# LiChaiUSTC/Speech-enhancement-based-on-a-maximum-likelihood-criterion

Hardware: AMD Instinct MI355X
Metric: training frames/sec (128-frame minibatch) (higher is better)
Workload: dtype f32

## Files before the change

### speech-enhancement-based-on-a-maximum-likelihood-criterion_amd/__init__.py

```python
import collections
import ctypes as C
import os
import subprocess

import numpy as np

_HERE = os.path.dirname(os.path.abspath(__file__))
_CSRC = os.path.join(_HERE, "csrc")
LIB_PATH = os.path.join(_CSRC, "libmlggd.so")
MAXLAYER = 10
UNIQUE_ID_BYTES = 128

_fp = C.POINTER(C.c_float)
_fpp = C.POINTER(_fp)


class MlggdError(RuntimeError):
    pass


class _ConfigSlots(C.Union):
    _fields_ = [("mask_bins", C.c_int32), ("reserved", C.c_int32 * 5)]


# ... 32 lines not shown
    "mlggd_debug_stamp_select", "mlggd_debug_stamp_read",
    "mlggd_load_frames", "mlggd_train_frames", "mlggd_train_frames_async", "mlggd_cv_all_frames", "mlggd_forward_frames",
    "mlggd_alloc_pinned", "mlggd_alloc_pinned_on", "mlggd_free_pinned", "mlggd_set_cv_device_reduce",
    "mlggd_comm_info", "mlggd_debug_plan_count", "mlggd_debug_buffers", "mlggd_debug_math", "mlggd_debug_out_slabs", "mlggd_debug_gemm_plan",
    "mlggd_debug_keep_ranks", "mlggd_debug_rank_tensor",
    "mlggd_wave_to_lps", "mlggd_lps_to_wave", "mlggd_enhance_wave",
    "mlggd_enhance_waves_layout", "mlggd_enhance_waves",
    "mlggd_score_waves", "mlggd_enhance_waves_scored",
    "mlggd_stoi_layout", "mlggd_stoi_waves", "mlggd_enhance_waves_scored_stoi",
    "mlggd_live_layout", "mlggd_live_open", "mlggd_live_push", "mlggd_live_received", "mlggd_live_close",
    "mlggd_error_stats", "mlggd_error_stats_frames", "mlggd_ggd_fit",
    "mlggd_set_shapefactors", "mlggd_get_shapefactors", "mlggd_read_shapefactors",
    "mlggd_output_stats", "mlggd_output_stats_frames", "mlggd_gv_fit", "mlggd_set_gv", "mlggd_get_gv", "mlggd_read_gv",
    "mlggd_wave_samples", "mlggd_mix_waves", "mlggd_lps_stats", "mlggd_norm_from_stats",
    "mlggd_load_waves", "mlggd_cv_all_waves", "mlggd_set_noise", "mlggd_train_waves",
    "mlggd_load_frames_nat", "mlggd_train_frames_nat", "mlggd_cv_all_frames_nat", "mlggd_forward_frames_nat",
    "mlggd_nat_estimate", "mlggd_nat_rows", "mlggd_get_nat_frames",
    "mlggd_set_mask", "mlggd_get_mask", "mlggd_get_mask_bins", "mlggd_mask_targets", "mlggd_mask_select",
    "mlggd_set_asymmetry", "mlggd_get_asymmetry", "mlggd_error_stats_signed", "mlggd_error_stats_signed_frames",
    "mlggd_asym_fit", "mlggd_read_asymmetry",
    "mlggd_set_scale_mode", "mlggd_get_scale_mode", "mlggd_get_scale_state", "mlggd_set_scale_state",
    "mlggd_read_scale_state", "mlggd_write_scale_state",
    "mlggd_rbm_open", "mlggd_rbm_set_rates", "mlggd_rbm_train_chunk", "mlggd_rbm_train_frames", "mlggd_rbm_visible_bias",
    "mlggd_rbm_debug_tensor", "mlggd_rbm_close", "mlggd_rbm_draws",
]
MAX_BETAS = 32

_lib = None


def build(force=False):
    srcs = [os.path.join(_CSRC, f) for f in ("engine.hip", "kernels.hip.h", "kernels64.hip.h", "spectral.hip.h", "score.hip.h", "live.hip.h",
                                             "live_rule.h", "stoi.hip.h", "stoi_rule.h", "colstats.hip.h", "gv_rule.h", "mask_rule.h", "mask.hip.h", "mix.hip.h",
                                             "mix_rule.h", "nat_rule.h", "rbm_rule.h", "rbm.hip.h", "asym_rule.h", "scale_rule.h", "devbuf.h", "devbuf_rule.h")]
    srcs.append(os.path.join(_HERE, "..", "include", "mlggd.h"))
    srcs.append(os.path.join(_HERE, "host", "errmodel.h"))
    srcs.append(os.path.join(_HERE, "host", "gvfile.h"))
    srcs.append(os.path.join(_HERE, "host", "asymfile.h"))
    srcs.append(os.path.join(_HERE, "host", "scalefile.h"))
    srcs.append(os.path.join(_HERE, "host", "binfile.h"))
    stale = not os.path.exists(LIB_PATH) or any(
        os.path.getmtime(LIB_PATH) < os.path.getmtime(s) for s in srcs)
    if force or stale:
        subprocess.check_call(["make", "-C", _CSRC, "-s"])
    return LIB_PATH


def load():
    global _lib
    if _lib is not None:
        return _lib
    if not os.path.exists(LIB_PATH):
        raise MlggdError("HIP extension %s is missing: run __graft_entry__.build() "
                         "(there is no CPU fallback)" % LIB_PATH)
    L = C.CDLL(LIB_PATH)
    L.mlggd_last_error.restype = C.c_char_p
    L.mlggd_gamma.restype = C.c_float
    L.mlggd_gamma.argtypes = [C.c_float]
    L.mlggd_create.argtypes = [C.POINTER(_Config), _fpp, _fpp, C.POINTER(C.c_void_p)]
    L.mlggd_destroy.argtypes = [C.c_void_p]
    L.mlggd_device_count.argtypes = [C.POINTER(C.c_int)]
    L.mlggd_train_chunk.argtypes = [C.c_void_p, C.c_int, _fp, _fp, C.POINTER(C.c_int)]
    L.mlggd_load_chunk.argtypes = [C.c_void_p, C.c_int, _fp, _fp]
    L.mlggd_train_resident.argtypes = [C.c_void_p, C.c_int, C.c_int, C.POINTER(C.c_int)]
    L.mlggd_sync.argtypes = [C.c_void_p]
    for f in (L.mlggd_cv_sqerr, L.mlggd_cv_abserr, L.mlggd_cv_loglik):
        f.argtypes = [C.c_void_p, C.c_int, _fp, _fp, _fp]
# ... 1291 lines not shown
```

### speech-enhancement-based-on-a-maximum-likelihood-criterion_amd/csrc/engine.hip

```cpp
#include <hip/hip_runtime.h>
#include <hip/hip_ext.h>

#include <dlfcn.h>
#include <math.h>
#include <stdarg.h>
#include <stdio.h>
#include <stdlib.h>
#include <string.h>

#include <algorithm>
#include <functional>
#include <mutex>
#include <string>
#include <vector>

#include "../../include/mlggd.h"
#include "../host/errmodel.h"
#include "../host/gvfile.h"
#include "../host/asymfile.h"
#include "../host/scalefile.h"
#include "kernels.hip.h"
#include "spectral.hip.h"
#include "score.hip.h"
#include "stoi.hip.h"
// ... 247 lines not shown
    int ar_shard = 1;
    hipEvent_t ev_grad[MLGGD_MAXLAYER] = {0}, ev_red[MLGGD_MAXLAYER] = {0}, ev_bias = nullptr, ev_bias_red = nullptr;

    hipEvent_t ev_t0 = nullptr, ev_t1 = nullptr;
    int last_steps = 0;
    bool timing_valid = false;
    int prof_class = -1, prof_layer = 0, prof_stride = 1;
    std::vector<hipEvent_t> prof_ev;
    size_t prof_used = 0, prof_cap = 0;
    hipEvent_t *prof_attach = nullptr;
    bool prof_attached = false;
    hipEvent_t stop_ev_next = nullptr;
    bool stop_ev_attached = false;
    int dp_stopev = 1;
    double prof_flops = 0, prof_bytes = 0;

    int stamp_class = -1, stamp_layer = 0, stamp_blocks = 0;
    DevBuf<long long> stamp_buf;

    struct DwpTable {
        DwpJobs key;
        bool fused;
        int grid;
        DevBuf<DwpDesc> dev;
    };
    std::vector<DwpTable> dwp_tables;
    std::vector<void *> allocs;
    std::vector<const void *> lds_attr_done;

    int mask_bins = 0;
    int mask_mode = mask_rule::kSelect;
    float mask_lo = mask_rule::kLo, mask_hi = mask_rule::kHi, mask_scale = mask_rule::kScale;
    int rbm_open = 0;
};

static long long *stamps_for(mlggd_engine *e, int cls, int layer, int blocks) {
    if (e->stamp_class != cls || e->stamp_layer != layer || !e->stamp_buf.p) return nullptr;
    if ((size_t)blocks * 8 > e->stamp_buf.cap) return nullptr;
    e->stamp_class = -1;
    e->stamp_blocks = blocks;
    return e->stamp_buf.p;
}

struct DevBufs {
    std::vector<void *> p;
    ~DevBufs() {
        for (void *q : p) hipFree(q);
    }
    template <typename T>
    int alloc(T **out, size_t count) {
        void *q = nullptr;
        HIPCHK(hipMalloc(&q, (count ? count : 1) * sizeof(T)));
        p.push_back(q);
        *out = (T *)q;
        return MLGGD_OK;
    }
    template <typename T>
    int upload(T **out, const T *host, size_t count) {
        CHK(alloc(out, count));
        if (count) HIPCHK(hipMemcpy(*out, host, count * sizeof(T), hipMemcpyHostToDevice));
        return MLGGD_OK;
    }
};

static int dev_alloc(mlggd_engine *e, float **p, size_t count) {
    const size_t bytes = (count + 64) * sizeof(float);
// ... 411 lines not shown
        if (a.Np >= (1 << 17)) return fail(MLGGD_ERR_ARG, "dW tile table: layer of %d units is too wide", a.Np);
        for (int tl = 0; tl < a.ntiles; tl++, n++) {
            const int kt = a.k_first + tl / a.n_wg, nt = tl % a.n_wg;
            const int k0 = kt * 64, n0 = nt * 64;
            DwpDesc &d = recs[n];
            d.A = a.Yrow + (k0 - a.k_base);
            d.Bm = a.dEdX + n0;
            const size_t base = (size_t)k0 * a.Np + n0;
            int rows = a.K - k0;
            rows = rows < 0 ? 0 : rows > 64 ? 64 : rows;
            if (a.wd_off) {
                rows = 0;
                d.W = a.Wt;
                d.D = a.delta;
                d.szW = 0;
            } else {
                d.W = (fused ? a.Wt : a.G) + base;
                d.D = fused ? a.delta + base : nullptr;
                const size_t to_end = ((size_t)a.Kp * a.Np - base) * sizeof(float);
                const size_t to_row = (size_t)rows * a.Np * sizeof(float);
                d.szW = (unsigned)(to_end < to_row ? to_end : to_row);
            }
            const int colsw = a.Np - n0 < 64 ? a.Np - n0 : 64;
            int nbias = (a.do_bias && kt == 0) ? a.N - n0 : 0;
            nbias = nbias < 0 ? 0 : nbias > 64 ? 64 : nbias;
            d.bias = (fused ? a.bias : a.gb) + n0;
            d.dbias = fused ? a.dbias + n0 : nullptr;
            d.ldA = a.ldA;
            d.Np = a.Np;
            d.packed = (unsigned)rows | ((unsigned)colsw << 8) | ((unsigned)nbias << 16) | (1u << 24);
        }
    }
    if (n != (size_t)J.total) return fail(MLGGD_ERR_STATE, "dW tile table: %zu records for %d tiles", n, J.total);
    for (; n < recs.size(); n++) {
        DwpDesc &d = recs[n];
        d = recs[0];
        d.packed = 0;
        d.szW = 0;
    }
    mlggd_engine::DwpTable t;
    t.key = key;
    t.fused = fused;
    t.grid = grid;
    HIPCHK(t.dev.grow(recs.size(), recs.size(), e->bufs, nullptr, nullptr));
    HIPCHK(hipMemcpy(t.dev.p, recs.data(), recs.size() * sizeof(DwpDesc), hipMemcpyHostToDevice));
    *out = t.dev.p;
    e->dwp_tables.push_back(std::move(t));
    return MLGGD_OK;
}

template <int H>
static int launch_dwp_t(mlggd_engine *e, const DwpJobs &J, bool fused, hipStream_t st, int stamp_layer) {
    const size_t lds = dwp_lds_floats() * sizeof(float);
    const int grid = dwp_grid(e, J.total);
    if (J.total < 1) return MLGGD_OK;
    const DwpDesc *table = nullptr;
    DwpConst C;
    C.B = J.job[0].B;
    C.nf = J.job[0].nf;
    C.mom = J.job[0].mom;
    C.lr = J.job[0].lr;
    C.wc = J.job[0].wc;
    bool bias_only = J.njobs > 0, any_bias_only = false;
    for (int j = 0; j < J.njobs; j++) {
        bias_only = bias_only && J.job[j].wd_off != 0;
        any_bias_only = any_bias_only || J.job[j].wd_off != 0;
    }
    if (any_bias_only) {
        if (!bias_only || !fused) return fail(MLGGD_ERR_STATE, "bias-only jobs need a launch of their own on the fused path");
        CHK(dwp_table(e, J, fused, grid, &table));
        unsigned nb;
        memcpy(&nb, &C.nf, sizeof(nb));
        if ((nb & 0x007FFFFFu) == 0u && C.nf >= 1.0f) {
            CHK(ensure_lds(e, k_dwp_bias<H, true>, lds));
            hipLaunchKernelGGL((k_dwp_bias<H, true>), dim3(grid), dim3(256), lds, st, table, J.total, C, (long long *)nullptr);
        } else {
            CHK(ensure_lds(e, k_dwp_bias<H, false>, lds));
            hipLaunchKernelGGL((k_dwp_bias<H, false>), dim3(grid), dim3(256), lds, st, table, J.total, C, (long long *)nullptr);
        }
        return launch_check("k_dwp_bias");
    }
    CHK(dwp_table(e, J, fused, grid, &table));
    if constexpr (H == 2 || H == 8) {
        if (e->stamp_class == KC_DW && e->stamp_layer == -1 && e->stamp_buf.p && fused && C.nf == 128.0f) {
            long long *sp = stamps_for(e, KC_DW, -1, 2 * grid);
            if (sp) {
                CHK(ensure_lds(e, k_dwp_phases<H>, lds));
                hipLaunchKernelGGL((k_dwp_phases<H>), dim3(grid), dim3(256), lds, st, table, J.total, C, sp);
                return launch_check("k_dwp_phases");
            }
        }
    }
    if constexpr (H == 2) {
        static const int abl = getenv("MLGGD_DWP_ABLATE") ? atoi(getenv("MLGGD_DWP_ABLATE")) : 0;
        if (abl && fused) {
#define DWP_ABL(A_)                                                                                       \
    case A_:                                                                                              \
        CHK(ensure_lds(e, k_dwp_ablate<H, A_>, lds));                                                     \
        launch_timed(e, k_dwp_ablate<H, A_>, dim3(grid), dim3(256), lds, st, table, J.total, C, (long long *)nullptr); \
        return launch_check("k_dwp_ablate");
            switch (abl) {
                DWP_ABL(1) DWP_ABL(2) DWP_ABL(3) DWP_ABL(4) DWP_ABL(7) DWP_ABL(15) DWP_ABL(31) DWP_ABL(63) DWP_ABL(16) DWP_ABL(48) DWP_ABL(256) DWP_ABL(1024) DWP_ABL(2048) DWP_ABL(512) DWP_ABL(576)
            default: return fail(MLGGD_ERR_ARG, "MLGGD_DWP_ABLATE=%d is not built", abl);
            }
#undef DWP_ABL
        }
    }
    long long *stamps = stamps_for(e, KC_DW, stamp_layer, grid);
    unsigned nfbits;
    memcpy(&nfbits, &C.nf, sizeof(nfbits));
    const bool pow2 = (nfbits & 0x007FFFFFu) == 0u && C.nf >= 1.0f;
#define DWP_LAUNCH(FUSED_, POW2_)                                                                         \
    {                                                                                                     \
        if (stamps) {                                                                                     \
            CHK(ensure_lds(e, k_dwp<H, FUSED_, POW2_, true>, lds));                                       \
            launch_timed(e, k_dwp<H, FUSED_, POW2_, true>, dim3(grid), dim3(256), lds, st, table, J.total, C, stamps); \
        } else {                                                                                          \
            CHK(ensure_lds(e, k_dwp<H, FUSED_, POW2_>, lds));                                             \
            launch_timed(e, k_dwp<H, FUSED_, POW2_>, dim3(grid), dim3(256), lds, st, table, J.total, C, stamps); \
        }                                                                                                 \
    }
    if (fused && pow2) DWP_LAUNCH(true, true)
    else if (fused) DWP_LAUNCH(true, false)
    else if (pow2) DWP_LAUNCH(false, true)
    else DWP_LAUNCH(false, false)
#undef DWP_LAUNCH
    return launch_check("k_dwp");
}
static bool dwp_usable(const mlggd_engine *e) {
    const int Hh = e->Bp / 64;
    return e->dw_persist && e->Bp % 64 == 0 && (Hh == 1 || Hh == 2 || Hh == 4 || Hh == 8);
}
static int launch_dwp(mlggd_engine *e, const DwpJobs &J, bool fused, hipStream_t st, int stamp_layer, int units = 0) {
    switch (units > 0 ? units : e->Bp / 64) {
    case 1: return launch_dwp_t<1>(e, J, fused, st, stamp_layer);
    case 2: return launch_dwp_t<2>(e, J, fused, st, stamp_layer);
    case 4: return launch_dwp_t<4>(e, J, fused, st, stamp_layer);
    case 8: return launch_dwp_t<8>(e, J, fused, st, stamp_layer);
    case 16: return launch_dwp_t<16>(e, J, fused, st, stamp_layer);
    default: return fail(MLGGD_ERR_STATE, "no dW kernel for %d units per tile", units);
    }
}

static bool gather_usable(const mlggd_engine *e, int world) {
    const long frames = (long)world * e->Bp;
    const long units = frames / 64;
    return e->dw_persist && e->B == e->Bp && frames % 64 == 0 &&
           (units == 1 || units == 2 || units == 4 || units == 8 || units == 16);
}
static int gather_alloc(mlggd_engine *e) {
    const size_t rows = (size_t)e->world * e->Bp;
    for (int l = 0; l < e->L - 1; l++) {
        const size_t width = e->dp_a2a ? (size_t)e->shard_rows[l + 1] * 64 : (size_t)e->lsp[l];
        CHK(dev_alloc(e, &e->Yall[l], rows * width));
        if (e->dp_a2a) {
            if (l == 0) {
                CHK(dev_alloc(e, &e->in_bunch_buf[0], rows * width));
                CHK(dev_alloc(e, &e->in_bunch_buf[1], rows * width));
                e->in_bunch = e->in_bunch_buf[0];
// ... 732 lines not shown
    if (ceil32(cfg->bunchsize) > 1152)
        return fail(MLGGD_ERR_ARG, "bunchsize %d too large for the loss kernel's LDS tile (max 1152)", cfg->bunchsize);
    int ndev = 0;
    hipError_t de = hipGetDeviceCount(&ndev);
    if (de != hipSuccess || ndev < 1)
        return fail(MLGGD_ERR_DEVICE, "no HIP device available (%s)", de == hipSuccess ? "count 0" : hipGetErrorString(de));
    if (cfg->device < 0 || cfg->device >= ndev)
        return fail(MLGGD_ERR_ARG, "GPU Num %d Not In Range %d-%d", cfg->device, 0, ndev - 1);

    mlggd_engine *e = new mlggd_engine();
    e->cfg = *cfg;
    e->L = cfg->numlayers;
    e->device = cfg->device;
    for (int i = 0; i < e->L; i++) {
        e->ls[i] = cfg->layersizes[i];
        e->lsp[i] = ceil32(cfg->layersizes[i]);
    }
    e->B = cfg->bunchsize;
    e->Bp = ceil32(e->B);
    e->K0 = e->ls[0];
    e->D = e->ls[e->L - 1];
    e->Dp = e->lsp[e->L - 1];
    e->nat_frames = cfg->nat_frames;
    e->mask_bins = cfg->mask_bins;
    if (const char *v = getenv("MLGGD_FWD_NW")) e->fwd_nw = atoi(v);
    if (const char *v = getenv("MLGGD_WAVES_LOOKUP")) e->ww.lookup_table = !strcmp(v, "table");
    if (const char *v = getenv("MLGGD_DX_NW")) e->dx_nw = atoi(v);
    if (const char *v = getenv("MLGGD_FWD_PIPE")) e->fwd_pipe = atoi(v);
    if (const char *v = getenv("MLGGD_DX_PIPE")) e->dx_pipe = atoi(v);
    if (const char *v = getenv("MLGGD_DW_TILE")) e->dw_tile = atoi(v);
    if (const char *v = getenv("MLGGD_TWO_STREAMS")) e->two_streams = atoi(v);
    if (const char *v = getenv("MLGGD_DW_PERSIST")) e->dw_persist = atoi(v);
    if (const char *v = getenv("MLGGD_DWP_PER_CU")) e->dwp_per_cu = atoi(v);
    if (const char *v = getenv("MLGGD_DW_MERGE")) e->dw_merge = atoi(v);
    if (const char *v = getenv("MLGGD_LOSS_FUSE")) e->loss_fuse = atoi(v);
    if (const char *v = getenv("MLGGD_TILE_MAP")) e->tile_map = atoi(v);
    if (const char *v = getenv("MLGGD_STAGE_AHEAD")) e->stage_ahead = atoi(v);
    if (const char *v = getenv("MLGGD_CV_DEVICE")) e->cv_device = atoi(v) ? 1 : 0;
    if (const char *v = getenv("MLGGD_TILE64")) e->tile64 = atoi(v);
    *out = e;

    roctx_load();
    HIPCHK(hipSetDevice(e->device));
    {
        int cus = 0;
        if (hipDeviceGetAttribute(&cus, hipDeviceAttributeMultiprocessorCount, e->device) == hipSuccess && cus > 0) e->n_cus = cus;
    }
    HIPCHK(hipStreamCreateWithFlags(&e->stream, hipStreamNonBlocking));
    if (e->two_streams) HIPCHK(hipStreamCreateWithFlags(&e->dw_stream, hipStreamNonBlocking));
    for (int l = 0; l < e->L; l++) HIPCHK(hipEventCreateWithFlags(&e->ev_dx[l], hipEventDisableTiming));
    HIPCHK(hipEventCreateWithFlags(&e->ev_upd, hipEventDisableTiming));
    HIPCHK(hipEventCreate(&e->ev_t0));
    HIPCHK(hipEventCreate(&e->ev_t1));

    const int L = e->L, Bp = e->Bp;
    CHK(dev_alloc(e, &e->Yt[0], (size_t)e->lsp[0] * Bp));
    CHK(dev_alloc(e, &e->in_bunch_buf[0], (size_t)(Bp + 1) * e->lsp[0]));
    CHK(dev_alloc(e, &e->in_bunch_buf[1], (size_t)(Bp + 1) * e->lsp[0]));
    e->in_bunch = e->in_bunch_buf[0];
    for (int l = 1; l < L; l++) {
        const size_t wsz = (size_t)e->lsp[l - 1] * e->lsp[l];
        CHK(dev_alloc(e, &e->W[l], wsz));
        CHK(dev_alloc(e, &e->dW[l], wsz));
        CHK(dev_alloc(e, &e->bias[l], e->lsp[l]));
        CHK(dev_alloc(e, &e->dbias[l], e->lsp[l]));
        const size_t asz = (size_t)e->lsp[l] * Bp;
        if (l != L - 1) {
            CHK(dev_alloc(e, &e->Yt[l], asz));
            CHK(dev_alloc(e, &e->Y[l], asz));
        }
        CHK(dev_alloc(e, &e->dEdXt[l], asz));
        CHK(dev_alloc(e, &e->dEdX[l], asz));
    }
    {
        const int tiles = (e->Dp / 32) * (Bp / 32);
        const int pairs = e->lsp[L - 2] / 2;
        int S = 256 / tiles >= 4 ? 256 / tiles : (256 + tiles - 1) / tiles;
        if (S > pairs / 16) S = pairs / 16;
        if (S < 1) S = 1;
        if (S > 32) S = 32;
        if (const char *v = getenv("MLGGD_S_OUT")) S = atoi(v) < 1 ? 1 : atoi(v) > 32 ? 32 : atoi(v);
        e->S_out = S;
    }
    CHK(dev_alloc(e, &e->slab, (size_t)e->S_out * e->Dp * Bp));
    CHK(dev_alloc(e, &e->outT, (size_t)e->Dp * Bp));
    CHK(dev_alloc(e, &e->eT, (size_t)e->Dp * Bp));
    CHK(dev_alloc(e, &e->pT, (size_t)e->Dp * Bp));
    CHK(dev_alloc(e, &e->colsum, e->Dp));
    CHK(dev_alloc(e, &e->scalefactor, e->Dp));

    const int rc = mlggd_set_weights(e, weights, bias);
    if (rc != MLGGD_OK) return rc;
    HIPCHK(hipStreamSynchronize(e->stream));
    return MLGGD_OK;
}

int mlggd_destroy(mlggd_handle e) {
    if (!e) return MLGGD_OK;
    if (e->live_groups > 0)
        return fail(MLGGD_ERR_STATE, "%d live group(s) of this engine are open: mlggd_live_close them first",
                    e->live_groups);
    if (e->rbm_open > 0) return fail(MLGGD_ERR_STATE, "an RBM session of this engine is open: mlggd_rbm_close it first");
    hipSetDevice(e->device);
    if (e->stream) hipStreamSynchronize(e->stream);
    if (e->comm_stream) hipStreamSynchronize(e->comm_stream);
    if (e->dw_stream) hipStreamSynchronize(e->dw_stream);
    if (e->stat_comm && g_rccl.CommDestroy) g_rccl.CommDestroy(e->stat_comm);
    if (e->comm && g_rccl.CommDestroy) g_rccl.CommDestroy(e->comm);
    for (void *p : e->allocs) hipFree(p);
    if (e->copy_stream) hipStreamSynchronize(e->copy_stream);
    for (auto &r : e->raw)
        if (r.last_use) hipEventDestroy(r.last_use);
    if (e->copy_stream) hipStreamDestroy(e->copy_stream);
    for (hipEvent_t ev : e->prof_ev) hipEventDestroy(ev);
    for (int l = 0; l < MLGGD_MAXLAYER; l++) {
        if (e->ev_grad[l]) hipEventDestroy(e->ev_grad[l]);
        if (e->ev_red[l]) hipEventDestroy(e->ev_red[l]);
    }
    for (int l = 0; l < MLGGD_MAXLAYER; l++) {
        if (e->ev_W[l]) hipEventDestroy(e->ev_W[l]);
        if (e->ev_layer[l]) hipEventDestroy(e->ev_layer[l]);
    }
// ... 2872 lines not shown
```

### speech-enhancement-based-on-a-maximum-likelihood-criterion_amd/csrc/kernels.hip.h

```cpp
#pragma once
#include <hip/hip_runtime.h>
#include "nat_rule.h"
#include "asym_rule.h"
#include "scale_rule.h"

typedef float f32x16 __attribute__((ext_vector_type(16)));
typedef float f32x2 __attribute__((ext_vector_type(2)));

__device__ __forceinline__ f32x16 mfma32(float a, float b, f32x16 c) {
    return __builtin_amdgcn_mfma_f32_32x32x2f32(a, b, c, 0, 0, 0);
}
__device__ __forceinline__ int acc_row(int r, int lane) { return (r & 3) + 8 * (r >> 2) + 4 * (lane >> 5); }

__device__ __forceinline__ void divmod_by(int x, int d, int shift, int &q, int &r) {
    if (shift >= 0) {
        q = x >> shift;
        r = x & (d - 1);
    } else {
        q = (int)((unsigned)x / (unsigned)d);
        r = x - q * d;
    }
}
__device__ __forceinline__ void tile_of_block(int id, int u_tiles, int b_tiles, int b_shift, int &ut, int &bt, int map = 0) {
    if ((u_tiles & 7) == 0 && map != 2) {
        const int xcd = id & 7, slot = id >> 3;
        int q;
        divmod_by(slot, b_tiles, b_shift, q, bt);
        ut = map == 1 ? xcd * (u_tiles >> 3) + q : xcd + 8 * q;
    } else {
        divmod_by(id, b_tiles, b_shift, ut, bt);
    }
}

template <int U>
struct FragU {
    float a[U];
    float b[U];
// ... 1031 lines not shown
    DwpArgs job[DWP_MAXJOBS];
    int tile_end[DWP_MAXJOBS];
    int njobs, total;
};
constexpr int dwp_lds_floats() { return 2 * 8192; }

struct DwpDesc {
    const float *A;
    const float *Bm;
    float *W;
    float *D;
    float *bias;
    float *dbias;
    int ldA, Np;
    unsigned packed;
    unsigned szW;
};
static_assert(sizeof(DwpDesc) == 64, "four 16-byte quarters per record");
struct DwpRaw {
    unsigned w[16];
};
typedef unsigned u32x4 __attribute__((ext_vector_type(4)));
__device__ __forceinline__ DwpDesc dwp_decode(u32x4 v) {
    DwpRaw r;
#pragma unroll
    for (int q = 0; q < 4; q++)
#pragma unroll
        for (int c = 0; c < 4; c++) r.w[4 * q + c] = (unsigned)__builtin_amdgcn_readlane((int)v[c], q);
    return __builtin_bit_cast(DwpDesc, r);
}
struct DwpConst {
    int B;
    float nf, mom, lr, wc;
};

constexpr int DWP_UPDATE_FORM = 2048;
template <int H, bool FUSED, bool POW2, bool PHASES = false, int ABL = 0>
__device__ __forceinline__ void dwp_body(const DwpDesc *__restrict__ table, const int total, const DwpConst C, const int bid,
                                         const int nblocks, float *lds, long long *stamps) {
    stamp_clk(stamps, 0, bid);
    const int B = C.B;
    const float nf = C.nf, mom = C.mom, lr = C.lr, wc = C.wc;
    const float inv_nf = 1.0f / nf;
    constexpr unsigned OOB = 0x7F000000u;
    const int tid = threadIdx.x, lane = tid & 63, wave = wave_id();
    const int i = lane & 31, h5 = lane >> 5;
    const int wm = wave >> 1, wn = wave & 1;
    const int scol = tid & 15, srow = tid >> 4;
    const int ec = lane & 7, er = lane >> 3;

    f32x16 acc, accp;
#pragma unroll
    for (int r = 0; r < 16; r++) acc[r] = accp[r] = 0.0f;
    float4 ra[4], rb[4];
    float4 pw0[4], pd0[4], pw1[4], pd1[4];
#pragma unroll
    for (int q = 0; q < 4; q++) pw1[q] = pd1[q] = make_float4(0.f, 0.f, 0.f, 0.f);
    float bsum = 0.0f, bsum_p = 0.0f;

    int t = bid;
    const rsrc_t rT = make_rsrc(table, ((size_t)total + 2 * (size_t)nblocks) * sizeof(DwpDesc));
    const int voT = 16 * (lane & 3);
#define DWP_FETCH(TI) __builtin_bit_cast(u32x4, __builtin_amdgcn_raw_buffer_load_b128(rT, voT, (TI) * 64, 0))
    u32x4 tc_raw = DWP_FETCH(t), tn_raw = DWP_FETCH(t + nblocks), tp_raw = tc_raw, tnn_raw;
    DwpDesc tc = dwp_decode(tc_raw), tn = dwp_decode(tn_raw), tp = tc;
    tp.packed = 0;
    tp.szW = 0;

#define DWP_COLS(T) ((int)(((T).packed >> 8) & 0xFFu))
#define DWP_NBIAS(T) ((int)(((T).packed >> 16) & 0xFFu))
#define DWP_SZAB(T) ((((T).packed >> 24) & 1u) ? 0x7FFFFFFFu : 0u)
#define DWP_DIVN(x) (POW2 ? (x) * inv_nf : (x) / nf)
#define DWP_DIVN2(x) (POW2 ? (x) * inv2 : (x) / nf2)
    f32x2 mom2 = {mom, mom}, lr2 = {lr, lr}, wc2 = {wc, wc}, inv2 = {inv_nf, inv_nf}, nf2 = {nf, nf}, one2 = {1.0f, 1.0f};
    constexpr int UPD = (ABL & (256 | 1024 | 2048)) ? (ABL & (256 | 1024 | 2048)) : DWP_UPDATE_FORM;
    if (UPD == 1024) asm volatile("" : "+v"(mom2), "+v"(lr2), "+v"(wc2), "+v"(inv2), "+v"(nf2), "+v"(one2));
#define DWP_OFF0(T) ((32 * wn + 4 * ec) < DWP_COLS(T) ? (unsigned)(((32 * wm + er) * T.Np + 32 * wn + 4 * ec) * 4) : OOB)
#define DWP_OFF(BASE, T, IT) ((int)((BASE) + (unsigned)((IT) * 32 * T.Np)))
#define DWP_WRITE_UNIT(BUF)                                                                     \
    {                                                                                           \
        float *as = lds + (BUF)*8192, *bs = as + 4096;                                          \
        _Pragma("unroll") for (int q = 0; q < 4; q++) {                                         \
            *reinterpret_cast<float4 *>(as + (srow + 16 * q) * 64 + 4 * scol) = ra[q];          \
            *reinterpret_cast<float4 *>(bs + (srow + 16 * q) * 64 + 4 * scol) = rb[q];          \
        }                                                                                       \
    }
#define DWP_BIAS(BUF, HH)                                                                       \
    {                                                                                           \
        if (tid < DWP_NBIAS(tc)) {                                                              \
            const float *col = lds + (BUF)*8192 + 4096 + tid;                                   \
            int bend = B - 64 * (HH);                                                           \
            bend = bend < 64 ? bend : 64;                                                       \
                                                     \
            asm volatile("" : "+s"(bend));                                                      \
            int b = 0;                                                                          \
            if ((HH) == 0) {  \
                bsum = col[0];                                                                  \
// ... 65 lines not shown
#define DWP_PHASE(K)                                                                            \
    {                                                                                           \
        if (PHASES) {                                                                           \
            __builtin_amdgcn_sched_barrier(0);                                                  \
            const long long now_ = (long long)__builtin_amdgcn_s_memtime();                     \
            ph_sum[K] += now_ - ph_last;                                                        \
            ph_last = now_;                                                                     \
            __builtin_amdgcn_sched_barrier(0);                                                  \
        }                                                                                       \
    }
#define DWP_UNIT(HH, BUF, PW, PD)                                                               \
    {                                                                                           \
        const bool FIRSTU = (HH) == 0, LASTU = (HH) == H - 1;  \
        DWP_BIAS(BUF, HH)                                                                       \
        if (FIRSTU) DWP_BIAS_UPDATE()                                                           \
                                        \
        const rsrc_t rA_ = LASTU ? make_rsrc(tn.A, DWP_SZAB(tn)) : make_rsrc(tc.A, DWP_SZAB(tc)); \
        const rsrc_t rB_ = LASTU ? make_rsrc(tn.Bm, DWP_SZAB(tn)) : make_rsrc(tc.Bm, DWP_SZAB(tc)); \
        const int ldA_ = LASTU ? tn.ldA : tc.ldA, ldB_ = LASTU ? tn.Np : tc.Np;                 \
        const int row0_ = LASTU ? 0 : 64 * ((HH) + 1);                                          \
                \
        const int voA_ = (srow * ldA_ + 4 * scol) * 4, voB_ = (srow * ldB_ + 4 * scol) * 4;     \
        const rsrc_t rWn = make_rsrc(tn.W, tn.szW), rDn = make_rsrc(tn.D, FUSED ? tn.szW : 0);  \
        const rsrc_t rWp = make_rsrc(tp.W, tp.szW), rDp = make_rsrc(tp.D, FUSED ? tp.szW : 0);  \
        const unsigned offp_ = FIRSTU ? DWP_OFF0(tp) : 0u, offn_ = (FUSED && LASTU) ? DWP_OFF0(tn) : 0u; \
        const float *ap = lds + (BUF)*8192 + h5 * 64 + 32 * wm + i;                             \
        const float *bp = lds + (BUF)*8192 + 4096 + h5 * 64 + 32 * wn + i;                      \
        float fa[32], fb[32];                               \
        float4 gq[4];                                                                           \
        _Pragma("unroll") for (int p = 0; p < 4; p++) {                                         \
            fa[p] = (ABL & 8) ? 1.0f : ap[p * 128];                                             \
            fb[p] = (ABL & 8) ? 1.0f : bp[p * 128];                                             \
        }                                                                                       \
        if (FIRSTU) tnn_raw = DWP_FETCH(t + 2 * nblocks);                                       \
        __builtin_amdgcn_sched_barrier(0);                                                      \
        _Pragma("unroll") for (int g = 0; g < 16; g++) {                                        \
            if (!(ABL & 12)) {                                                                  \
                acc = mfma32(fa[2 * g], fb[2 * g], acc);                                        \
                acc = mfma32(fa[2 * g + 1], fb[2 * g + 1], acc);                                \
            } else if (!(ABL & 8)) {                                                            \
                asm volatile("" ::"v"(fa[2 * g]), "v"(fb[2 * g]), "v"(fa[2 * g + 1]), "v"(fb[2 * g + 1])); \
            }                                                                                   \
            if (g < 14 && !(ABL & 8)) {                                                         \
                _Pragma("unroll") for (int p = 2 * g + 4; p < 2 * g + 6; p++) {                 \
                    fa[p] = ap[p * 128];                                                        \
                    fb[p] = bp[p * 128];                                                        \
                }                                                                               \
            }                                                                                   \
                      \
                                \
            if (!(ABL & 512) && !(ABL & 16)) {                                                  \
                const int qa = FIRSTU ? g - 6 : g, qb = FIRSTU ? g : g - 4;                     \
                if (qa >= 0 && qa < 4) {                                                        \
                    float *dst = lds + ((BUF) ^ 1) * 8192 + (4 * wave + 16 * qa) * 64;          \
                    __builtin_amdgcn_raw_ptr_buffer_load_lds(rA_, (__attribute__((address_space(3))) void *)dst, 16, \
                                                             voA_, (row0_ + 16 * qa) * ldA_ * 4, 0, 0);  \
                }                                                                               \
                if (qb >= 0 && qb < 4) {                                                        \
                    float *dst = lds + ((BUF) ^ 1) * 8192 + 4096 + (4 * wave + 16 * qb) * 64;   \
                    __builtin_amdgcn_raw_ptr_buffer_load_lds(rB_, (__attribute__((address_space(3))) void *)dst, 16, \
                                                             voB_, (row0_ + 16 * qb) * ldB_ * 4, 0, 0);  \
                }                                                                               \
            }                                                                                   \
            if ((ABL & 512) && !(ABL & 16) && (FIRSTU ? g < 4 : g < 8)) {                        \
                const bool two_ = FIRSTU;                                                       \
                const int q = two_ ? g : g >> 1, row = row0_ + srow + 16 * q;                    \
                if (two_ || (g & 1) == 0) ra[q] = bload4(rA_, (row * ldA_ + 4 * scol) * 4, 0);   \
// ... 17 lines not shown
                        PD[g - 12] = bload4(rDn, DWP_OFF(offn_, tn, g - 12), 0);                \
                    }                                                                           \
                } else if (g >= 8) {                                                            \
                    if (g < 12) PW[g - 8] = bload4(rWn, DWP_OFF(offn_, tn, g - 8), 0);          \
                    else PD[g - 12] = bload4(rDn, DWP_OFF(offn_, tn, g - 12), 0);               \
                }                                                                               \
            }                                                                                   \
             \
            if ((ABL & 512) && !(ABL & (32 | 64)) && g >= 12) {                                 \
                float *as_ = lds + ((BUF) ^ 1) * 8192, *bs_ = as_ + 4096;                       \
                *reinterpret_cast<float4 *>(as_ + (srow + 16 * (g - 12)) * 64 + 4 * scol) = ra[g - 12]; \
                *reinterpret_cast<float4 *>(bs_ + (srow + 16 * (g - 12)) * 64 + 4 * scol) = rb[g - 12]; \
            }                                                                                   \
            __builtin_amdgcn_sched_barrier(0);                                                  \
        }                                                                                       \
        DWP_PHASE(LASTU ? 2 : 0)                                                                \
        if ((ABL & 64) && !(ABL & 32)) DWP_WRITE_UNIT((BUF) ^ 1)                                \
        if (!(ABL & 512)) {                                                                     \
                             \
            constexpr int lo_ = 0;                                                              \
            const int younger = FIRSTU ? ((FUSED ? 2 : 1) + ((LASTU && FUSED) ? 8 : 0)) : ((LASTU && FUSED) ? 8 : 0); \
            if (younger == 0) __builtin_amdgcn_s_waitcnt(0x0F70 | lo_);                         \
            else if (younger == 1) __builtin_amdgcn_s_waitcnt(0x0F71);                          \
            else if (younger == 2) __builtin_amdgcn_s_waitcnt(0x0F72);                          \
            else if (younger == 8) __builtin_amdgcn_s_waitcnt(0x0F78);                          \
            else if (younger == 9) __builtin_amdgcn_s_waitcnt(0x0F79);                          \
            else __builtin_amdgcn_s_waitcnt(0x0F7A);                                            \
        }                                                                                       \
        __syncthreads();                                                                        \
        DWP_PHASE(LASTU ? 4 : 1)                                                                \
    }
#define DWP_TILE(BASE, PW, PD)                                                                  \
    {                                                                                           \
        _Pragma("unroll") for (int hh = 0; hh < H; hh++) DWP_UNIT(hh, ((BASE) + hh) & 1, PW, PD) \
         \
        accp = acc;                                                                             \
        _Pragma("unroll") for (int r = 0; r < 16; r++) acc[r] = 0.0f;                           \
        bsum_p = bsum;                                                                          \
        tp = tc;                                                                                \
        tp_raw = tc_raw;                                                                        \
        t += nblocks;                                                                           \
        if (t >= total) break;                                                                  \
        tc = tn;                                                                                \
        tc_raw = tn_raw;                                                                        \
        tn = dwp_decode(tnn_raw);                                                               \
        tn_raw = tnn_raw;                                                                       \
    }

    {
        const rsrc_t rA_ = make_rsrc(tc.A, DWP_SZAB(tc)), rB_ = make_rsrc(tc.Bm, DWP_SZAB(tc));
        const rsrc_t rWc = make_rsrc(tc.W, tc.szW), rDc = make_rsrc(tc.D, FUSED ? tc.szW : 0);
        const unsigned offc_ = DWP_OFF0(tc);
#pragma unroll
        for (int q = 0; q < 4; q++) {
            const int row = srow + 16 * q;
            ra[q] = bload4(rA_, (row * tc.ldA + 4 * scol) * 4, 0);
            rb[q] = bload4(rB_, (row * tc.Np + 4 * scol) * 4, 0);
        }
#pragma unroll
        for (int q = 0; q < 4; q++) {
            pw0[q] = FUSED ? bload4(rWc, DWP_OFF(offc_, tc, q), 0) : make_float4(0.f, 0.f, 0.f, 0.f);
            pd0[q] = FUSED ? bload4(rDc, DWP_OFF(offc_, tc, q), 0) : make_float4(0.f, 0.f, 0.f, 0.f);
        }
    }
    DWP_WRITE_UNIT(0)
    __syncthreads();
    if (PHASES) ph_last = (long long)__builtin_amdgcn_s_memtime();
    bool last_set1 = true;
    for (;;) {
        last_set1 = false;
        DWP_TILE(0, pw1, pd1)
        last_set1 = true;
        DWP_TILE(H & 1, pw0, pd0)
    }
    {
        DWP_BIAS_UPDATE()
        const rsrc_t rWp = make_rsrc(tp.W, tp.szW), rDp = make_rsrc(tp.D, FUSED ? tp.szW : 0);
        const unsigned offp_ = DWP_OFF0(tp);
        float4 gq[4];
        DWP_EPI_SCRATCH_WRITE(0, 0, 16)
        __builtin_amdgcn_wave_barrier();
        _Pragma("unroll") for (int it = 0; it < 4; it++) DWP_EPI_SCRATCH_READ(0, it)
        if (last_set1) {
            _Pragma("unroll") for (int it = 0; it < 4; it++) DWP_EPI_UPDATE(pw1, pd1, it)
        } else {
            _Pragma("unroll") for (int it = 0; it < 4; it++) DWP_EPI_UPDATE(pw0, pd0, it)
        }
    }
    stamp_clk(stamps, 2, bid);
    if (stamps != nullptr && threadIdx.x == 0) stamps[(size_t)bid * 8 + 4] = (t - bid) / nblocks;
    if (PHASES && stamps != nullptr && threadIdx.x == 0) {
#pragma unroll
        for (int k = 0; k < 5; k++) stamps[(size_t)(nblocks + bid) * 8 + k] = ph_sum[k];
    }
#undef DWP_PHASE
#undef DWP_FETCH
#undef DWP_WRITE_UNIT
#undef DWP_OFF
#undef DWP_OFF0
#undef DWP_BIAS
#undef DWP_BIAS_UPDATE
#undef DWP_EPI_SCRATCH_WRITE
#undef DWP_EPI_SCRATCH_READ
#undef DWP_EPI_UPDATE
#undef DWP_UNIT
#undef DWP_TILE
#undef DWP_COLS
#undef DWP_NBIAS
#undef DWP_SZAB
#undef DWP_DIVN
#undef DWP_DIVN2
}

extern __shared__ __attribute__((aligned(16))) float g_dyn_lds[];

template <int MODE, int NW, int PIPE = 1, bool STAMPED = false>
__global__ __launch_bounds__(64 * NW) void k_fwd(FwdArgs A, long long *stamps) {
    fwd_body<MODE, NW, PIPE>(A, (int)blockIdx.x, g_dyn_lds, STAMPED ? stamps : nullptr);
}
template <int NW, int PIPE = 1, int ACT = ACT_SIGMOID, bool STAMPED = false>
__global__ __launch_bounds__(64 * NW) void k_dx(DxArgs A, long long *stamps) {
    dx_body<NW, PIPE, ACT>(A, (int)blockIdx.x, g_dyn_lds, STAMPED ? stamps : nullptr);
}
#include "kernels64.hip.h"
template <int H, bool FUSED, bool POW2, bool STAMPED = false>
__global__ __launch_bounds__(256) void k_dwp(const DwpDesc *__restrict__ table, int total, DwpConst C, long long *stamps) {
    dwp_body<H, FUSED, POW2>(table, total, C, (int)blockIdx.x, (int)gridDim.x, g_dyn_lds, STAMPED ? stamps : nullptr);
}
template <int H, bool POW2>
__global__ __launch_bounds__(256) void k_dwp_bias(const DwpDesc *__restrict__ table, int total, DwpConst C, long long *stamps) {
    dwp_body<H, true, POW2, false, 15>(table, total, C, (int)blockIdx.x, (int)gridDim.x, g_dyn_lds, nullptr);
}
template <int H, int ABL>
__global__ __launch_bounds__(256) void k_dwp_ablate(const DwpDesc *__restrict__ table, int total, DwpConst C, long long *stamps) {
    dwp_body<H, true, true, false, ABL>(table, total, C, (int)blockIdx.x, (int)gridDim.x, g_dyn_lds, nullptr);
}
template <int H>
__global__ __launch_bounds__(256) void k_dwp_phases(const DwpDesc *__restrict__ table, int total, DwpConst C, long long *stamps) {
    dwp_body<H, true, true, true>(table, total, C, (int)blockIdx.x, (int)gridDim.x, g_dyn_lds, stamps);
}
__global__ __launch_bounds__(256) void k_apply_update(float *__restrict__ Wt, float *__restrict__ delta,
                                                      const float *__restrict__ G, size_t n4, float nf, float mom,
                                                      float lr, float wc) {
    const size_t stride = (size_t)gridDim.x * blockDim.x;
    for (size_t idx = (size_t)blockIdx.x * blockDim.x + threadIdx.x; idx < n4; idx += stride) {
        const float4 g = reinterpret_cast<const float4 *>(G)[idx];
        float4 w = reinterpret_cast<float4 *>(Wt)[idx];
        float4 d = reinterpret_cast<float4 *>(delta)[idx];
        d.x = mom * d.x - lr * (g.x / nf + wc * w.x);
        d.y = mom * d.y - lr * (g.y / nf + wc * w.y);
        d.z = mom * d.z - lr * (g.z / nf + wc * w.z);
        d.w = mom * d.w - lr * (g.w / nf + wc * w.w);
        w.x = d.x + 1.0f * w.x;
        w.y = d.y + 1.0f * w.y;
        w.z = d.z + 1.0f * w.z;
        w.w = d.w + 1.0f * w.w;
        reinterpret_cast<float4 *>(delta)[idx] = d;
        reinterpret_cast<float4 *>(Wt)[idx] = w;
    }
}
// ... 742 lines not shown
```

Before: 1.058 million.

## Balance bias tiles across dW blocks and add atomic tail-tile claiming

```diff
diff --git a/speech-enhancement-based-on-a-maximum-likelihood-criterion_amd/__init__.py b/speech-enhancement-based-on-a-maximum-likelihood-criterion_amd/__init__.py
--- a/speech-enhancement-based-on-a-maximum-likelihood-criterion_amd/__init__.py
+++ b/speech-enhancement-based-on-a-maximum-likelihood-criterion_amd/__init__.py
@@ -88,7 +88,7 @@
 def build(force=False):
     srcs = [os.path.join(_CSRC, f) for f in ("engine.hip", "kernels.hip.h", "kernels64.hip.h", "spectral.hip.h", "score.hip.h", "live.hip.h",
                                              "live_rule.h", "stoi.hip.h", "stoi_rule.h", "colstats.hip.h", "gv_rule.h", "mask_rule.h", "mask.hip.h", "mix.hip.h",
-                                             "mix_rule.h", "nat_rule.h", "rbm_rule.h", "rbm.hip.h", "asym_rule.h", "scale_rule.h", "devbuf.h", "devbuf_rule.h")]
+                                             "mix_rule.h", "nat_rule.h", "rbm_rule.h", "rbm.hip.h", "asym_rule.h", "scale_rule.h", "dwp_rule.h", "devbuf.h", "devbuf_rule.h")]
     srcs.append(os.path.join(_HERE, "..", "include", "mlggd.h"))
     srcs.append(os.path.join(_HERE, "host", "errmodel.h"))
     srcs.append(os.path.join(_HERE, "host", "gvfile.h"))
diff --git a/speech-enhancement-based-on-a-maximum-likelihood-criterion_amd/csrc/dwp_rule.h b/speech-enhancement-based-on-a-maximum-likelihood-criterion_amd/csrc/dwp_rule.h
--- /dev/null
+++ b/speech-enhancement-based-on-a-maximum-likelihood-criterion_amd/csrc/dwp_rule.h
@@ -0,0 +1,104 @@
+#pragma once
+#include <stddef.h>
+
+#include <vector>
+
+#if defined(__HIPCC__)
+#define DWP_HD __host__ __device__
+#else
+#define DWP_HD
+#endif
+
+namespace dwp_rule {
+
+constexpr int kMaxStreams = 8;
+constexpr int kCounterStride = 16;
+
+struct Split {
+    int n, S, R;
+};
+DWP_HD inline Split split(int total, int grid) {
+    Split s;
+    s.n = total / grid;
+    s.S = s.n * grid;
+    s.R = total - s.S;
+    return s;
+}
+DWP_HD inline unsigned pool_index(unsigned old, unsigned base) { return old - base; }
+DWP_HD inline int pool_record(unsigned idx, int S, int R) { return idx < (unsigned)R ? S + (int)idx : -1; }
+DWP_HD inline int claimed_record(unsigned old, unsigned base, int S, int R) { return pool_record(pool_index(old, base), S, R); }
+DWP_HD inline int claim_position(int n) { return n >= 3 ? n - 3 : -1; }
+DWP_HD inline unsigned advance(unsigned base, int grid) { return base + (unsigned)grid; }
+
+struct Counters {
+    const void *stream[kMaxStreams] = {nullptr};
+    unsigned next[kMaxStreams] = {0};
+    int used = 0;
+    int slot(const void *st) {
+        for (int i = 0; i < used; i++)
+            if (stream[i] == st) return i;
+        if (used == kMaxStreams) return -1;
+        stream[used] = st;
+        next[used] = 0;
+        return used++;
+    }
+    unsigned take(int s, int grid) {
+        const unsigned base = next[s];
+        next[s] = advance(base, grid);
+        return base;
+    }
+};
+
+inline std::vector<int> order(int total, int grid, const std::vector<char> &bias) {
+    std::vector<int> perm((size_t)total);
+    for (int r = 0; r < total; r++) perm[(size_t)r] = r;
+    if (grid < 1 || total < grid) return perm;
+    const Split sp = split(total, grid);
+    int nbias = 0;
+    for (int r = 0; r < total; r++) nbias += bias[(size_t)r] ? 1 : 0;
+    const int cap = (nbias + grid - 1) / grid;
+    std::vector<int> held((size_t)grid, 0);
+    auto is_bias = [&](int pos) { return bias[(size_t)perm[(size_t)pos]] != 0; };
+    std::vector<char> counted((size_t)grid);
+    for (int p = 0; p < sp.n; p++) {
+        counted.assign((size_t)grid, 0);
+        for (int w = 0; w < grid; w++) {
+            const int pos = p * grid + w;
+            if (!is_bias(pos) || counted[(size_t)w]) continue;
+            if (held[(size_t)w] < cap) {
+                held[(size_t)w]++;
+                continue;
+            }
+            int to = -1;
+            for (int d = 1; d < grid && to < 0; d++) {
+                const int v = (w + d) % grid;
+                if (!is_bias(p * grid + v) && held[(size_t)v] < cap) to = v;
+            }
+            if (to < 0) {
+                held[(size_t)w]++;
+                continue;
+            }
+            const int other = p * grid + to;
+            const int r = perm[(size_t)pos];
+            perm[(size_t)pos] = perm[(size_t)other];
+            perm[(size_t)other] = r;
+            held[(size_t)to]++;
+            counted[(size_t)to] = 1;
+        }
+    }
+    for (int pos = sp.S; pos < total; pos++) {
+        if (!is_bias(pos)) continue;
+        int to = -1;
+        for (int p = sp.n - 1; p >= 0 && to < 0; p--)
+            for (int w = 0; w < grid && to < 0; w++)
+                if (!is_bias(p * grid + w) && held[(size_t)w] < cap) to = p * grid + w;
+        if (to < 0) break;
+        const int r = perm[(size_t)pos];
+        perm[(size_t)pos] = perm[(size_t)to];
+        perm[(size_t)to] = r;
+        held[(size_t)(to % grid)]++;
+    }
+    return perm;
+}
+
+}
diff --git a/speech-enhancement-based-on-a-maximum-likelihood-criterion_amd/csrc/engine.hip b/speech-enhancement-based-on-a-maximum-likelihood-criterion_amd/csrc/engine.hip
--- a/speech-enhancement-based-on-a-maximum-likelihood-criterion_amd/csrc/engine.hip
+++ b/speech-enhancement-based-on-a-maximum-likelihood-criterion_amd/csrc/engine.hip
@@ -303,6 +303,9 @@
     int mask_mode = mask_rule::kSelect;
     float mask_lo = mask_rule::kLo, mask_hi = mask_rule::kHi, mask_scale = mask_rule::kScale;
     int rbm_open = 0;
+    int dwp_claim = 0, dwp_order = 1;
+    DevBuf<unsigned> dwp_counters;
+    dwp_rule::Counters dwp_ctr;
 };
 
 static long long *stamps_for(mlggd_engine *e, int cls, int layer, int blocks) {
@@ -780,6 +783,21 @@
         }
     }
     if (n != (size_t)J.total) return fail(MLGGD_ERR_STATE, "dW tile table: %zu records for %d tiles", n, J.total);
+    if (e->dwp_order && grid <= J.total) {
+        std::vector<char> is_bias((size_t)J.total);
+        bool any = false, all = true;
+        for (int r = 0; r < J.total; r++) {
+            is_bias[(size_t)r] = ((recs[(size_t)r].packed >> 16) & 0xFFu) != 0;
+            any = any || is_bias[(size_t)r];
+            all = all && is_bias[(size_t)r];
+        }
+        if (any && !all) {
+            const std::vector<int> perm = dwp_rule::order(J.total, grid, is_bias);
+            std::vector<DwpDesc> moved((size_t)J.total);
+            for (int pos = 0; pos < J.total; pos++) moved[(size_t)pos] = recs[(size_t)perm[(size_t)pos]];
+            std::copy(moved.begin(), moved.end(), recs.begin());
+        }
+    }
     for (; n < recs.size(); n++) {
         DwpDesc &d = recs[n];
         d = recs[0];
@@ -809,6 +827,9 @@
     C.mom = J.job[0].mom;
     C.lr = J.job[0].lr;
     C.wc = J.job[0].wc;
+    C.base = 0;
+    C.nstat = 0;
+    C.claim = nullptr;
     bool bias_only = J.njobs > 0, any_bias_only = false;
     for (int j = 0; j < J.njobs; j++) {
         bias_only = bias_only && J.job[j].wd_off != 0;
@@ -858,21 +879,36 @@
     unsigned nfbits;
     memcpy(&nfbits, &C.nf, sizeof(nfbits));
     const bool pow2 = (nfbits & 0x007FFFFFu) == 0u && C.nf >= 1.0f;
+    const dwp_rule::Split sp = dwp_rule::split(J.total, grid);
+    const bool wanted = e->dwp_claim == 2 || (e->dwp_claim == 1 && dwp_rule::claim_position(sp.n) >= 0);
+    const int slot = (wanted && sp.R > 0 && e->dwp_counters.p) ? e->dwp_ctr.slot((const void *)st) : -1;
+    const bool claim = slot >= 0;
+    if (claim) {
+        C.nstat = sp.n;
+        C.claim = e->dwp_counters.p + (size_t)slot * dwp_rule::kCounterStride;
+        C.base = e->dwp_ctr.take(slot, grid);
+    }
+#define DWP_LAUNCH_C(FUSED_, POW2_, CLAIM_)                                                               \
+    {                                                                                                     \
+        if (stamps) {                                                                                     \
+            CHK(ensure_lds(e, k_dwp<H, FUSED_, POW2_, true, CLAIM_>, lds));                               \
+            launch_timed(e, k_dwp<H, FUSED_, POW2_, true, CLAIM_>, dim3(grid), dim3(256), lds, st, table, J.total, C, stamps); \
+        } else {                                                                                          \
+            CHK(ensure_lds(e, k_dwp<H, FUSED_, POW2_, false, CLAIM_>, lds));                              \
+            launch_timed(e, k_dwp<H, FUSED_, POW2_, false, CLAIM_>, dim3(grid), dim3(256), lds, st, table, J.total, C, stamps); \
+        }                                                                                                 \
+    }
 #define DWP_LAUNCH(FUSED_, POW2_)                                                                         \
     {                                                                                                     \
-        if (stamps) {                                                                                     \
-            CHK(ensure_lds(e, k_dwp<H, FUSED_, POW2_, true>, lds));                                       \
-            launch_timed(e, k_dwp<H, FUSED_, POW2_, true>, dim3(grid), dim3(256), lds, st, table, J.total, C, stamps); \
-        } else {                                                                                          \
-            CHK(ensure_lds(e, k_dwp<H, FUSED_, POW2_>, lds));                                             \
-            launch_timed(e, k_dwp<H, FUSED_, POW2_>, dim3(grid), dim3(256), lds, st, table, J.total, C, stamps); \
-        }                                                                                                 \
+        if (claim) DWP_LAUNCH_C(FUSED_, POW2_, true)                                                      \
+        else DWP_LAUNCH_C(FUSED_, POW2_, false)                                                           \
     }
     if (fused && pow2) DWP_LAUNCH(true, true)
     else if (fused) DWP_LAUNCH(true, false)
     else if (pow2) DWP_LAUNCH(false, true)
     else DWP_LAUNCH(false, false)
 #undef DWP_LAUNCH
+#undef DWP_LAUNCH_C
     return launch_check("k_dwp");
 }
 static bool dwp_usable(const mlggd_engine *e) {
@@ -1671,6 +1707,8 @@
     if (const char *v = getenv("MLGGD_TWO_STREAMS")) e->two_streams = atoi(v);
     if (const char *v = getenv("MLGGD_DW_PERSIST")) e->dw_persist = atoi(v);
     if (const char *v = getenv("MLGGD_DWP_PER_CU")) e->dwp_per_cu = atoi(v);
+    if (const char *v = getenv("MLGGD_DWP_CLAIM")) e->dwp_claim = atoi(v) == 2 ? 2 : atoi(v) ? 1 : 0;
+    if (const char *v = getenv("MLGGD_DWP_ORDER")) e->dwp_order = atoi(v) ? 1 : 0;
     if (const char *v = getenv("MLGGD_DW_MERGE")) e->dw_merge = atoi(v);
     if (const char *v = getenv("MLGGD_LOSS_FUSE")) e->loss_fuse = atoi(v);
     if (const char *v = getenv("MLGGD_TILE_MAP")) e->tile_map = atoi(v);
@@ -1727,6 +1765,10 @@
     CHK(dev_alloc(e, &e->pT, (size_t)e->Dp * Bp));
     CHK(dev_alloc(e, &e->colsum, e->Dp));
     CHK(dev_alloc(e, &e->scalefactor, e->Dp));
+    {
+        const size_t n = (size_t)dwp_rule::kMaxStreams * dwp_rule::kCounterStride;
+        HIPCHK(e->dwp_counters.grow(n, n, e->bufs, &e->stream, nullptr));
+    }
 
     const int rc = mlggd_set_weights(e, weights, bias);
     if (rc != MLGGD_OK) return rc;
diff --git a/speech-enhancement-based-on-a-maximum-likelihood-criterion_amd/csrc/kernels.hip.h b/speech-enhancement-based-on-a-maximum-likelihood-criterion_amd/csrc/kernels.hip.h
--- a/speech-enhancement-based-on-a-maximum-likelihood-criterion_amd/csrc/kernels.hip.h
+++ b/speech-enhancement-based-on-a-maximum-likelihood-criterion_amd/csrc/kernels.hip.h
@@ -3,6 +3,7 @@
 #include "nat_rule.h"
 #include "asym_rule.h"
 #include "scale_rule.h"
+#include "dwp_rule.h"
 
 typedef float f32x16 __attribute__((ext_vector_type(16)));
 typedef float f32x2 __attribute__((ext_vector_type(2)));
@@ -1100,10 +1101,13 @@
 struct DwpConst {
     int B;
     float nf, mom, lr, wc;
+    unsigned base;
+    int nstat;
+    unsigned *claim;
 };
 
 constexpr int DWP_UPDATE_FORM = 2048;
-template <int H, bool FUSED, bool POW2, bool PHASES = false, int ABL = 0>
+template <int H, bool FUSED, bool POW2, bool PHASES = false, int ABL = 0, bool CLAIM = false>
 __device__ __forceinline__ void dwp_body(const DwpDesc *__restrict__ table, const int total, const DwpConst C, const int bid,
                                          const int nblocks, float *lds, long long *stamps) {
     stamp_clk(stamps, 0, bid);
@@ -1130,7 +1134,41 @@
     const rsrc_t rT = make_rsrc(table, ((size_t)total + 2 * (size_t)nblocks) * sizeof(DwpDesc));
     const int voT = 16 * (lane & 3);
 #define DWP_FETCH(TI) __builtin_bit_cast(u32x4, __builtin_amdgcn_raw_buffer_load_b128(rT, voT, (TI) * 64, 0))
-    u32x4 tc_raw = DWP_FETCH(t), tn_raw = DWP_FETCH(t + nblocks), tp_raw = tc_raw, tnn_raw;
+    __shared__ unsigned claim_lds[4];
+    const int t_stat = bid + (CLAIM ? C.nstat : 0) * nblocks;
+#define DWP_NONE (t_stat + nblocks)
+    int extra = DWP_NONE, nbias_walked = 0;
+    unsigned claim_old = 0;
+    if (CLAIM && tid == 0) {
+        claim_lds[0] = C.base;
+        claim_lds[1] = (unsigned)(total - (t_stat - bid));
+        *reinterpret_cast<unsigned long long *>(&claim_lds[2]) = (unsigned long long)C.claim;
+    }
+#define DWP_CLAIM_ISSUE()                                                                       \
+    {                                                                                           \
+        if (tid == 0) {                                                                         \
+             \
+            unsigned long long ctr_ = *reinterpret_cast<const unsigned long long *>(&claim_lds[2]); \
+            asm volatile("" : "+v"(ctr_));                                                      \
+            claim_old = __hip_atomic_fetch_add((__attribute__((address_space(1))) unsigned *)ctr_, 1u, __ATOMIC_RELAXED, \
+                                               __HIP_MEMORY_SCOPE_AGENT);                       \
+        }                                                                                       \
+    }
+#define DWP_CLAIM_TAKE()                                                                        \
+    {                                                                                           \
+        if (tid == 0) claim_lds[0] = dwp_rule::pool_index(claim_old, claim_lds[0]);             \
+        __syncthreads();                                                                        \
+        const int rec_ = dwp_rule::pool_record((unsigned)__builtin_amdgcn_readfirstlane((int)claim_lds[0]), t_stat - bid, \
+                                               __builtin_amdgcn_readfirstlane((int)claim_lds[1])); \
+        if (rec_ >= 0) extra = rec_;                                                            \
+    }
+#define DWP_REC(TQ) ((TQ) < t_stat ? (TQ) : (TQ) == t_stat ? extra : DWP_NONE)
+#define DWP_CLAIM_HERE() (t + 3 * nblocks == t_stat)
+    if (CLAIM && t_stat - bid < 3 * nblocks) {
+        DWP_CLAIM_ISSUE()
+        DWP_CLAIM_TAKE()
+    }
+    u32x4 tc_raw = DWP_FETCH(t), tn_raw = DWP_FETCH(CLAIM ? DWP_REC(t + nblocks) : t + nblocks), tp_raw = tc_raw, tnn_raw;
     DwpDesc tc = dwp_decode(tc_raw), tn = dwp_decode(tn_raw), tp = tc;
     tp.packed = 0;
     tp.szW = 0;
@@ -1262,7 +1300,8 @@
             fa[p] = (ABL & 8) ? 1.0f : ap[p * 128];                                             \
             fb[p] = (ABL & 8) ? 1.0f : bp[p * 128];                                             \
         }                                                                                       \
-        if (FIRSTU) tnn_raw = DWP_FETCH(t + 2 * nblocks);                                       \
+                                            \
+        if (FIRSTU) tnn_raw = DWP_FETCH(CLAIM ? DWP_REC(t + 2 * nblocks) : t + 2 * nblocks);    \
         __builtin_amdgcn_sched_barrier(0);                                                      \
         _Pragma("unroll") for (int g = 0; g < 16; g++) {                                        \
             if (!(ABL & 12)) {                                                                  \
@@ -1346,15 +1385,20 @@
     }
 #define DWP_TILE(BASE, PW, PD)                                                                  \
     {                                                                                           \
-        _Pragma("unroll") for (int hh = 0; hh < H; hh++) DWP_UNIT(hh, ((BASE) + hh) & 1, PW, PD) \
+        _Pragma("unroll") for (int hh = 0; hh < H; hh++) {                                      \
+            if (CLAIM && hh == H - 1 && DWP_CLAIM_HERE()) DWP_CLAIM_ISSUE()                     \
+            DWP_UNIT(hh, ((BASE) + hh) & 1, PW, PD)                                             \
+        }                                                                                       \
+        if (stamps != nullptr && !PHASES) nbias_walked += DWP_NBIAS(tc) > 0 ? 1 : 0;  \
          \
         accp = acc;                                                                             \
         _Pragma("unroll") for (int r = 0; r < 16; r++) acc[r] = 0.0f;                           \
         bsum_p = bsum;                                                                          \
         tp = tc;                                                                                \
         tp_raw = tc_raw;                                                                        \
+        if (CLAIM && DWP_CLAIM_HERE()) DWP_CLAIM_TAKE()                                         \
         t += nblocks;                                                                           \
-        if (t >= total) break;                                                                  \
+        if (t >= (CLAIM ? (extra != DWP_NONE ? DWP_NONE : t_stat) : total)) break;              \
         tc = tn;                                                                                \
         tc_raw = tn_raw;                                                                        \
         tn = dwp_decode(tnn_raw);                                                               \
@@ -1403,11 +1447,21 @@
     }
     stamp_clk(stamps, 2, bid);
     if (stamps != nullptr && threadIdx.x == 0) stamps[(size_t)bid * 8 + 4] = (t - bid) / nblocks;
+    if (!PHASES && stamps != nullptr && threadIdx.x == 0) {
+        stamps[(size_t)bid * 8 + 6] = (long long)__builtin_amdgcn_s_getreg(4 | (31 << 11)) |
+                                      ((long long)(__builtin_amdgcn_s_getreg(20 | (3 << 11)) & 0xF) << 32) | (1ll << 40);
+        stamps[(size_t)bid * 8 + 7] = (long long)(nbias_walked + 1) | ((long long)(CLAIM && extra != DWP_NONE ? extra + 1 : 0) << 32);
+    }
     if (PHASES && stamps != nullptr && threadIdx.x == 0) {
 #pragma unroll
         for (int k = 0; k < 5; k++) stamps[(size_t)(nblocks + bid) * 8 + k] = ph_sum[k];
     }
 #undef DWP_PHASE
+#undef DWP_CLAIM_ISSUE
+#undef DWP_CLAIM_TAKE
+#undef DWP_REC
+#undef DWP_NONE
+#undef DWP_CLAIM_HERE
 #undef DWP_FETCH
 #undef DWP_WRITE_UNIT
 #undef DWP_OFF
@@ -1437,9 +1491,10 @@
     dx_body<NW, PIPE, ACT>(A, (int)blockIdx.x, g_dyn_lds, STAMPED ? stamps : nullptr);
 }
 #include "kernels64.hip.h"
-template <int H, bool FUSED, bool POW2, bool STAMPED = false>
+template <int H, bool FUSED, bool POW2, bool STAMPED = false, bool CLAIM = false>
 __global__ __launch_bounds__(256) void k_dwp(const DwpDesc *__restrict__ table, int total, DwpConst C, long long *stamps) {
-    dwp_body<H, FUSED, POW2>(table, total, C, (int)blockIdx.x, (int)gridDim.x, g_dyn_lds, STAMPED ? stamps : nullptr);
+    dwp_body<H, FUSED, POW2, false, 0, CLAIM>(table, total, C, (int)blockIdx.x, (int)gridDim.x, g_dyn_lds,
+                                              STAMPED ? stamps : nullptr);
 }
 template <int H, bool POW2>
 __global__ __launch_bounds__(256) void k_dwp_bias(const DwpDesc *__restrict__ table, int total, DwpConst C, long long *stamps) {
```

New measurement: 1.050 million. No clear change (-0.8%).
